# MaaniGhaffari/cvo-rgbd

Measured on AMD Instinct MI355X. Metric: frame-pair registrations/sec, higher is better.
Workload: dtype f32; 1 GPU; BASELINE configs[1] shape: 64 distinct synthetic 10000x10000 RGB-D cloud pairs (xyz + 5-dim colour) per align_many call, cvo align() to convergence, clouds resident in HBM; points_fixed=10000, points_moving=10000, mode=cvo, batch=64

## Files before the change

### cvo-rgbd_amd/csrc/cvo_capi.cpp

```cpp
#include "cvo_internal.h"

using namespace cvo_dev;
using namespace cvo_impl;

namespace cvo_impl {

int fail(cvo_hip_ctx *ctx, int code, const char *msg)
{
    if (ctx) ctx->err = msg;
    return code;
}

static std::atomic<bool> g_engine_debug{false};
bool engine_debug_on() { return g_engine_debug.load(std::memory_order_relaxed); }

namespace {
struct OptDef {
    const char *key;
    const char *env;
    int env_kind;
    double env_value;
};
const OptDef kOptions[] = {
    {"graph_capture", "CVO_HIP_GRAPH", 1, 1.0},           {"no_graph", "CVO_HIP_NO_GRAPH", 1, 1.0},
// ... 4 lines not shown
    {"async_builds", "CVO_HIP_NO_ASYNC", 1, 0.0},         {"list_pass_blocks", "CVO_HIP_PROC_BLOCKS", 2, 0.0},
    {"post_debug", "CVO_HIP_POST_DEBUG", 1, 1.0},         {"mailbox_timeout_s", "CVO_HIP_MAILBOX_TIMEOUT_S", 2, 0.0},
    {"candidate_records", "CVO_HIP_NO_CAND", 1, 0.0},     {"sync_upload", "CVO_HIP_SYNC_UPLOAD", 1, 1.0},
    {"engine_debug", "CVO_HIP_ENGINE_DEBUG", 1, 1.0},     {"one_launch_hand_over", "CVO_HIP_NO_CLOUD_ONE", 1, 0.0},
    {"small_calls_alone", "CVO_HIP_NO_ALONE", 1, 0.0},    {"fused_groups", "CVO_HIP_NO_FUSE", 1, 0.0},
    {"engines", "CVO_HIP_ENGINES_FORCE", 2, 0.0},         {"list_init", "CVO_HIP_LIST_INIT", 2, 0.0},
    {"kept_pack", "CVO_HIP_NO_PACK", 1, 0.0},             {"list_margin", "CVO_HIP_LIST_MARGIN", 2, 0.0},
    {"final_mirror", "CVO_HIP_NO_FINAL_MIRROR", 1, 0.0},  {"twist_on_shared_gpu", "CVO_HIP_TWIST_ON_SHARED_GPU", 1, 1.0},
    {"comm_debug", "CVO_HIP_COMM_DEBUG", 1, 1.0},         {"wait_policy", "CVO_HIP_WAIT_POLICY", 2, 0.0},
    {"acvo_runs", "CVO_HIP_NO_ACVO_RUN", 1, 0.0},         {"tail_alone", "CVO_HIP_TAIL_ALONE", 2, 0.0},         {"side_builds", "CVO_HIP_SIDE", 1, 1.0},
    {"run_build_at", "CVO_HIP_RUN_BUILD_AT", 2, 0.0},         {"alone_max", "CVO_HIP_ALONE_MAX", 2, 0.0},
    {"narrow_merge", "CVO_HIP_NARROW_MERGE", 1, 1.0},     {"narrow_blocks", "CVO_HIP_NARROW_BLOCKS", 2, 0.0},
    {"engine_crowd", "CVO_HIP_ENGINE_CROWD", 2, 0.0},     {"engine_merge_max", "CVO_HIP_ENGINE_MERGE_MAX", 2, 0.0},
    {"matches_combine", nullptr, 0, 0.0},                 {"scan_chunk", nullptr, 0, 0.0},
    {"record_narrow", "CVO_HIP_NO_RECORD_NARROW", 1, 0.0}, {"list_stale_max", "CVO_HIP_LIST_STALE_MAX", 2, 0.0},
};
void env_defaults(cvo_hip_ctx *ctx)
{
    for (const OptDef &d : kOptions) {
        if (!d.env) continue;
        const char *e = getenv(d.env);
        if (!e) continue;
        (void)apply_option(ctx, d.key, d.env_kind == 1 ? d.env_value : atof(e));
    }
}
}

int apply_option(cvo_hip_ctx *ctx, const char *key, double v)
{
    auto is = [&](const char *k) { return std::strcmp(key, k) == 0; };
// ... 23 lines not shown
    else if (is("post_debug")) o.post_debug = on;
    else if (is("mailbox_timeout_s")) { if (!(v > 0.0)) return CVO_HIP_ERR_INVALID; o.mailbox_timeout_s = v; }
    else if (is("candidate_records")) o.no_cand = !on;
    else if (is("sync_upload")) o.sync_upload = on;
    else if (is("engine_debug")) { o.engine_debug = on; if (on) g_engine_debug.store(true, std::memory_order_relaxed); }
    else if (is("one_launch_hand_over")) o.no_cloud_one = !on;
    else if (is("small_calls_alone")) o.no_alone = !on;
    else if (is("fused_groups")) o.no_fuse = !on;
    else if (is("engines")) { if (v < 0.0 || v > 8.0) return CVO_HIP_ERR_INVALID; o.engines_force = (int)v; }
    else if (is("list_init")) { if (v < 0.0) return CVO_HIP_ERR_INVALID; o.list_init = v; }
    else if (is("kept_pack")) o.no_pack = !on;
    else if (is("matches_combine")) o.matches_combine = on;
    else if (is("scan_chunk")) { if (v < 0.0 || v > (double)SCAN_CHUNK) return CVO_HIP_ERR_INVALID; o.scan_chunk = (int)v; }
    else if (is("list_margin")) { if (v > 4.0) return CVO_HIP_ERR_INVALID; o.list_margin = v < 0.0 ? -1.0f : (float)v; }
    else if (is("record_narrow")) o.record_narrow = on;
    else if (is("list_stale_max")) { if (!(v >= 1.0 && v <= 64.0)) return CVO_HIP_ERR_INVALID; o.list_stale_max = (float)v; }
    else if (is("final_mirror")) o.no_final_mirror = !on;
    else if (is("twist_on_shared_gpu")) o.twist_on_shared_gpu = on;
    else if (is("comm_debug")) o.comm_debug = on;
    else if (is("wait_policy")) { if (v < 0.0 || v > 2.0) return CVO_HIP_ERR_INVALID; o.wait_policy = (int)v; }
    else if (is("acvo_runs")) o.no_acvo_run = !on;
    else if (is("tail_alone")) { if (v < 0.0 || v > 32.0) return CVO_HIP_ERR_INVALID; o.tail_alone = (int)v; }
    else if (is("run_restart")) o.no_restart = !on;
    else if (is("side_builds")) o.no_side_builds = !on;
    else if (is("run_build_at")) { if (!(v > 0.0 && v <= 1.0)) return CVO_HIP_ERR_INVALID; o.run_build_at = (float)v; }
    else if (is("alone_max")) { if (v < 0.0 || v > 64.0) return CVO_HIP_ERR_INVALID; o.alone_max = (int)v; }
    else if (is("narrow_merge")) o.narrow_merge = on;
    else if (is("narrow_blocks")) { const int b = (int)v; if (b != 0 && b != 32 && b != 64) return CVO_HIP_ERR_INVALID; o.narrow_blocks = b; }
    else if (is("engine_crowd")) { if (v < 0.0) return CVO_HIP_ERR_INVALID; o.engine_crowd = (int)std::min(v, 1.0e6); }
    else if (is("engine_merge_max")) { if (v < 0.0 || v > 32.0) return CVO_HIP_ERR_INVALID; o.engine_merge_max = (int)v; }
// ... 725 lines not shown
    else if (is("engine_debug")) *value = o.engine_debug;
    else if (is("one_launch_hand_over")) *value = !o.no_cloud_one;
    else if (is("small_calls_alone")) *value = !o.no_alone;
    else if (is("fused_groups")) *value = !o.no_fuse;
    else if (is("engines")) *value = o.engines_force;
    else if (is("narrow_merge")) *value = o.narrow_merge;
    else if (is("narrow_blocks")) *value = o.narrow_blocks;
    else if (is("engine_crowd")) *value = o.engine_crowd;
    else if (is("engine_merge_max")) *value = o.engine_merge_max;
    else if (is("list_init")) *value = o.list_init;
    else if (is("kept_pack")) *value = !o.no_pack;
    else if (is("matches_combine")) *value = o.matches_combine;
    else if (is("scan_chunk")) *value = o.scan_chunk;
    else if (is("list_margin")) *value = o.list_margin;
    else if (is("record_narrow")) *value = o.record_narrow;
    else if (is("list_stale_max")) *value = o.list_stale_max;
    else if (is("final_mirror")) *value = !o.no_final_mirror;
    else if (is("twist_on_shared_gpu")) *value = o.twist_on_shared_gpu;
    else if (is("comm_debug")) *value = o.comm_debug;
    else if (is("wait_policy")) *value = o.wait_policy;
    else if (is("acvo_runs")) *value = !o.no_acvo_run;
    else if (is("tail_alone")) *value = o.tail_alone;
    else if (is("tail_handovers")) *value = (double)ctx->tail_handovers;
    else if (is("run_restart")) *value = !o.no_restart;
    else if (is("side_builds")) *value = !o.no_side_builds;
    else if (is("run_build_at")) *value = o.run_build_at;
    else if (is("side_builds_launched")) *value = (double)ctx->side_builds_launched;
    else if (is("alone_max")) *value = o.alone_max;
    else if (is("run_timeouts")) *value = (double)ctx->run_timeouts;
    else if (is("list_grows")) *value = (double)ctx->list_grows;
    else if (is("async_builds_named")) *value = (double)ctx->async_stats[0];
    else if (is("async_stalls")) *value = (double)ctx->async_stats[1];
    else if (is("run_aborts")) *value = (double)ctx->run_aborts;
    else if (is("engine_begins")) *value = (double)ctx->engine_begins;
    else if (is("engine_final_mirrored")) *value = (double)ctx->engine_final_mirrored;
    else if (is("engine_final_copied")) *value = (double)ctx->engine_final_copied;
    else if (is("no_run_backoff")) *value = ctx->no_run_backoff;
    else return CVO_HIP_ERR_INVALID;
    return CVO_HIP_OK;
}

long long cvo_hip_get_mirror_retries(void) { return mirror_retries().load(std::memory_order_relaxed); }

int cvo_hip_synchronize(cvo_hip_ctx *ctx)
{
// ... 9 lines not shown
```

### cvo-rgbd_amd/csrc/cvo_device.h

```cpp
#pragma once

#include <hip/hip_runtime.h>
#include <hip/hip_ext.h>
#include <stddef.h>
#include <stdint.h>

#include "cvo_hip.h"
#include "se3_math.hpp"

namespace cvo_dev {

constexpr int FEAT_STRIDE = 8;
constexpr int FEAT_INDEX_SLOT = 5;

constexpr int BLOCK = 256;
constexpr int TILES_PER_WAVE = 4;
constexpr int ROWS_PER_WAVE = 16 * TILES_PER_WAVE;
constexpr int ROWS_PER_TILE = 4 * ROWS_PER_WAVE;
constexpr float PAD_BIG = 1.0e30f;
constexpr int PROC_BLOCKS = 1024;
constexpr int PROC_WAVES = PROC_BLOCKS * 4;

constexpr int NSUB = 256;
constexpr int PROC_PARTS = PROC_BLOCKS / NSUB;
constexpr int TILE_STAGE = 128;
constexpr int DEAL_SHIFT = 2;
constexpr int PAIR_QUEUE = 128;
constexpr int SEG = 64;
constexpr int MAX_CSEG = 32;

typedef uint4 TileEntry;

enum ProcMode { PROC_FLOW = 0, PROC_STEP = 1, PROC_SELF = 2 };
enum ListId { LIST_XY = 0, LIST_XX = 1, LIST_YY = 2, LIST_KEPT = 3, LIST_XYB = 4, LIST_XXB = 5, LIST_YYB = 6,
              LIST_N = 7 };
CVO_HD int self_list_id(int l, int buf) { return buf ? LIST_XXB + l : LIST_XX + l; }

constexpr int NACC_FLOW = 9;
constexpr int NACC_STEP = 4;
constexpr int NACC_SELF = 2;
constexpr int NACC_MAX = 9;

constexpr int RED_FLOW = 0, RED_XX = 9, RED_YY = 11, RED_STEP = 13, RED_N = 17;

enum { RUNNING = 0, DONE_BREAK_A = 1, DONE_BREAK_B = 2, DONE_MAX_ITER = 3, NEED_BIGGER_LIST = 4,
       DONE_COMM_ERROR = 5,
// ... 64 lines not shown
    int32_t mode, max_iter;
    float ell_init, ell_min, ell_max_init;
    float sp, c_sp;
    float c, d, c_ell;
    float min_step, eps, eps_2;
    float log_sp_s2;
    float tau_c;
    float list_margin;
    int32_t async_xy;
    float build_at;
    int32_t async_self;
    float color_scale;
    float run_cand_cap;
    int32_t record_narrow;
    float list_stale_max;
    double s2_d, cs2_d, dl_step;
};

struct alignas(16) DevHead {
    float R[9], T[3];
    float ell, ell_max;
    float Rt[9], t[3];
    float used_Rt[9], used_t[3];
    KernConsts kc;
    float kc_ell, kc_pad_;
    float center[3];
    float xmax, y0max;
    float tauf[3];
    int32_t n_fixed;
    uint32_t pad0_;
    float list_r[3];
    int32_t list_ok[3];
    int32_t reuse[3];
    int32_t ck_nblk[3];
    float list_Rt[9], list_t[3];
    float rec_r;
    int32_t narrow;
    float rec_Rt[9], rec_t[3];
    int32_t list_stat[3];
    int32_t async_stat[2];
    int32_t rec_pad_;
    int32_t xy_active, xy_target, stall, xy_fresh;
    int32_t xy_ok[2];
    int32_t xy_ck[2];
    float xy_r[2];
    float tauf_build;
    float r_last;
    float xy_Rt[2][9], xy_t[2][3];
    int32_t sf_active[2], sf_target[2], sf_fresh[2];
    int32_t sf_ok[2][2];
    int32_t sf_ck[2][2];
    float sf_r[2][2];
    float sf_tauf_build[2];
    cvo_math::XiConsts xi;
    float omega[3], v[3];
    double dl;
// ... 216 lines not shown
}
CVO_HD float cull_slack(const float *t, const float cx, const float cy, const float cz, const float xmax, const float y0max)
{
    const float W = ((fabsf(cx) + fabsf(cy)) + fabsf(cz)) + (xmax + y0max);
    return (64.0f / 16777216.0f) * (3.0003f * W + ((fabsf(t[0]) + fabsf(t[1])) + fabsf(t[2])));
}

CVO_HD float reuse_slack(const float *t, const float *c, const float xmax, const float y0max, const float sides)
{
    const float W = ((fabsf(c[0]) + fabsf(c[1])) + fabsf(c[2])) + (xmax + y0max);
    const float S = 3.0003f * W + ((fabsf(t[0]) + fabsf(t[1])) + fabsf(t[2]));
    return 1.0e-4f * (1.0f + xmax + y0max) + sides * (22.0f / 16777216.0f) * S;
}

constexpr float LIST_LOOSE = 1.3f;
CVO_HD float pose_travel(const DevHead *s, const float *Rt0, const float *t0, const float ymax)
{
    float f2 = 0.0f, c2 = 0.0f;
    for (int r = 0; r < 3; ++r) {
        float dc = s->t[r] - t0[r];
        for (int q = 0; q < 3; ++q) {
            const float d = s->Rt[3 * r + q] - Rt0[3 * r + q];
            f2 += d * d;
            dc += d * s->center[q];
        }
        c2 += dc * dc;
    }
    return sqrtf(0.5f * f2) * 1.001f * ymax + sqrtf(c2);
}
CVO_HD void plan_lists(DevHead *s, DevHead *bulk, const bool store, const DevParams &p, const float r_now)
{
    const float ymax = s->y0max;
    const float slack_xx = reuse_slack(s->t, s->center, s->xmax, ymax, 0.0f), slack_xy = reuse_slack(s->t, s->center, s->xmax, ymax, 1.0f);
    const float wide_yy = slack_xy - slack_xx;
    const float margin = p.list_margin;
    const bool sync_xy = s->list_ok[LIST_XY] && !p.async_xy;
    const float travel = sync_xy ? pose_travel(s, s->list_Rt, s->list_t, ymax) : 0.0f;
#pragma unroll
    for (int l = 0; l < 3; ++l) {
        if (l == LIST_XY && p.async_xy) continue;
        if (l != LIST_XY && p.async_self) continue;
        if (l != LIST_XY && p.mode != CVO_HIP_MODE_ACVO) { s->reuse[l] = 1; continue; }
        const float slack = l == LIST_XX ? slack_xx : slack_xy;
        const float need = (r_now + (l == LIST_XY ? travel : 0.0f)) * 1.0001f + slack;
        const float lr = s->list_r[l];
        const float r0 = r_now * 1.0001f + slack;
        const float rb = r0 * (1.0f + margin);
        bool keep = margin > 0.0f && s->list_ok[l] && need <= lr;
        if (l == LIST_XY && p.record_narrow && keep && s->ck_nblk[LIST_XY] != 0) {
            const float tr = pose_travel(s, s->rec_Rt, s->rec_t, ymax);
            const float rr = s->rec_r;
            keep = (r_now + tr) * 1.0001f + slack <= rr && lr <= fmaxf(p.list_stale_max, LIST_LOOSE) * (1.0f + margin) * r0;
            s->narrow &= REC_BOUNDED;
            if (keep && !(rr <= LIST_LOOSE * (1.0f + margin) * r0)) {
                keep = (rb + tr) * 1.0001f + slack <= rr;
                if (keep) {
                    s->rec_r = rb * 1.000001f;
                    s->narrow = REC_NARROW | REC_BOUNDED;
                    s->list_stat[1] += 1;
                    if (store) {
                        for (int q = 0; q < 9; ++q) bulk->rec_Rt[q] = s->Rt[q];
                        for (int q = 0; q < 3; ++q) bulk->rec_t[q] = s->t[q];
                    }
                }
            }
        } else {
            keep = keep && lr <= LIST_LOOSE * (1.0f + margin) * r0;
// ... 447 lines not shown
    const float4 *pos_b;
    const float *feat_b;
    const float4 *seg_b;
    const float *tf;
    double *partials;
    double *out;
    KernConsts kc;
    int nseg_a, nseg_b;
    int nblk;
    int count;
};
void launch_pose_scan(const ScanArgs &a, int weight, hipStream_t s);

void launch_prepare(DevState *st, const DevParams &prm, hipStream_t s, uint32_t *build_masks = nullptr, const PrepareInit *init = nullptr);
void launch_prepare_many(const PrepareEntry *e, int n, hipStream_t s, uint32_t *build_masks);
void launch_filter(const FilterArgs &a, dim3 grid, hipStream_t s, hipEvent_t ev_start = nullptr,
                   hipEvent_t ev_stop = nullptr);
void launch_process(int mode, const ProcessArgs &a, hipStream_t s, hipEvent_t ev_start = nullptr,
                    hipEvent_t ev_stop = nullptr);
void launch_post_flow(const PostFlowArgs &a, hipStream_t s);
void launch_post_step(const PostStepArgs &a, hipStream_t s);
void launch_filter_group(const FilterArgs *a, int n, hipStream_t s);
void launch_process_group(int mode, const ProcessArgs *a, int n, hipStream_t s, hipEvent_t ev_start = nullptr,
                          hipEvent_t ev_stop = nullptr);
void launch_post_flow_group(const PostFlowArgs *a, int n, hipStream_t s);
void launch_post_step_group(const PostStepArgs *a, int n, hipStream_t s);
void launch_step_twist_group(const ProcessArgs *a, int n, hipStream_t s, hipEvent_t ev_start = nullptr,
                             hipEvent_t ev_stop = nullptr);
constexpr int STEP_TWIST_ROWS_DIV = 4;

// ... 21 lines not shown
```

### cvo-rgbd_amd/csrc/cvo_engine.cpp

```cpp
#include "cvo_internal.h"

using namespace cvo_dev;
using namespace cvo_impl;

namespace cvo_impl {

bool fusable(const cvo_hip_ctx *c) { return !c->profiling && !multi_rank(c) && !(c->prm.color_scale > 0.0f); }



struct EngineProfile {
    std::mutex mu;
    bool on = false;
    double flow_ms = 0.0, flow_slots = 0.0;
    long long flow_launches = 0;
    std::vector<float> dur_us, period_us;
    std::vector<int> slots;
};
EngineProfile *engine_profile()
{
    static EngineProfile *p = new EngineProfile;
    return p;
}

// ... 30 lines not shown
    struct Retire { hipEvent_t ev = nullptr; std::vector<AlignJob *> jobs; };
    std::vector<Retire> retiring;
    hipEvent_t ev[4] = {};
    std::vector<PrepareEntry> prep;
    long long launched = 0, checked = 0;
    int zdim = 0;
    bool crowded = true, use_graph = true, dirty = true, failed = false;
    int batch_len = kEngineBatch;
    bool narrow = false;
    bool narrow_merge = false;
    int narrow_blocks = 0;
    bool wind_down = false;
    std::vector<TLaunch> plan;
    struct FlowEv { hipEvent_t a, b; int live; };
    std::vector<FlowEv> flow_ev;
    long long n_batches[5] = {}, n_replans = 0, n_inserts = 0, n_sends = 0, n_prepares = 0, n_mirrored = 0, n_copied = 0;
    double t_replan = 0, t_insert = 0, t_launch = 0, t_finish = 0, t_wait = 0, t_collect = 0, t_idle_at = 0;
    static double now_ms() { return std::chrono::duration<double, std::milli>(std::chrono::steady_clock::now().time_since_epoch()).count(); }

    int create(int dev)
    {
        device = dev;
        if (hipSetDevice(dev) != hipSuccess) return -1;
        if (hipStreamCreateWithFlags(&s, hipStreamNonBlocking) != hipSuccess) return -1;
        if (tab.init(ENGINE_SLOTS, s) != 0) return -1;
        for (auto &e : ev)
            if (hipEventCreateWithFlags(&e, hipEventDisableTiming) != hipSuccess) return -1;
        return 0;
    }

    int live() const { int n = 0; for (AlignJob *j : member) n += j != nullptr; return n; }
// ... 88 lines not shown
            return CVO_HIP_OK;
        }
        member[z] = j;
        ops[z].clear();
        dirty = true;
        return CVO_HIP_OK;
    }

    int replan()
    {
        int n = 0;
        for (int z = 0; z < ENGINE_SLOTS; ++z) n += member[z] != nullptr;
        int zd = 1;
        while (zd < n) zd *= 2;
        if (n > 16 && n <= 24) zd = 24;
        for (int z = ENGINE_SLOTS - 1, hole = 0; z >= zd; --z) {
            if (!member[z]) continue;
            while (member[hole]) ++hole;
            member[hole] = member[z]; member[z] = nullptr;
            ops[hole].swap(ops[z]); ops[z].clear();
        }
        const bool regeom = zd != zdim;
        zdim = zd;
        const int nblk = (narrow && narrow_blocks > 0) ? std::min(narrow_blocks, nblk_for(zdim)) : nblk_for(zdim);
        int merge_max = 2;
        std::vector<const std::vector<RecOp> *> po;
        std::vector<Slot *> ps;
        for (int z = 0; z < ENGINE_SLOTS; ++z)
            if (member[z]) { merge_max = member[z]->ctx->opt.engine_merge_max; break; }
        for (int z = 0; z < ENGINE_SLOTS; ++z) {
// ... 239 lines not shown
                if (q + 1 < e->flow_ev.size() && hipEventElapsedTime(&gap, fe.a, e->flow_ev[q + 1].a) != hipSuccess) gap = 0.f;
                if (pr->dur_us.size() < (size_t)1 << 20) {
                    pr->dur_us.push_back(ms * 1e3f); pr->period_us.push_back(gap * 1e3f); pr->slots.push_back(fe.live);
                }
            }
        }
        for (auto &fe : e->flow_ev) {
            (void)hipEventDestroy(fe.a);
            (void)hipEventDestroy(fe.b);
        }
        e->flow_ev.clear();
    }
    std::lock_guard<std::mutex> lock(*engine_mutex());
    if (engine_debug_on())
        fprintf(stderr, "[cvo_hip] engine %p: batches at zdim 1/2/4/8/16: %lld %lld %lld %lld %lld, replans %lld, "
                "prepare launches %lld, final states mirrored %lld copied %lld, graph captures %lld hits %lld; host ms: insert %.2f replan %.2f launch %.2f collect %.2f finish %.2f wait %.2f\n",
                (void *)e, e->n_batches[0], e->n_batches[1], e->n_batches[2],
                e->n_batches[3], e->n_batches[4], e->n_replans, e->n_prepares, e->n_mirrored, e->n_copied, e->plans.captures, e->plans.hits,
                e->t_insert, e->t_replan, e->t_launch, e->t_collect, e->t_finish, e->t_wait);
    e->t_insert = e->t_replan = e->t_launch = e->t_collect = e->t_finish = e->t_wait = 0;
    for (long long &v : e->n_batches) v = 0;
    e->n_replans = e->n_prepares = e->n_mirrored = e->n_copied = 0;
    e->launched = e->checked = 0;
    e->in_use = false;
}


}

extern "C" {

int cvo_hip_align_many(cvo_hip_ctx **ctxs, cvo_hip_state **states, int *n_iters, int count)
{
    cvo_lock::Api api_guard;
    if (count < 0 || (count > 0 && (!ctxs || !states))) return CVO_HIP_ERR_INVALID;
    const bool dbg_many = engine_debug_on();
    const double t_many0 = Engine::now_ms();
// ... 224 lines not shown
```

### cvo-rgbd_amd/csrc/cvo_internal.h

```cpp
#pragma once
#include "cvo_hip.h"

#include <hip/hip_runtime.h>

#include <algorithm>
#include <atomic>
#include <chrono>
#include <cmath>
#include <cstddef>
#include <cstdint>
#include <cstdio>
#include <cstdlib>
#include <cstring>
#include <deque>
#include <memory>
#include <mutex>
#include <new>
#include <string>
#include <thread>
#include <vector>

#include "cvo_cloud.h"
#include "cvo_comm.h"
#include "cvo_device.h"
// ... 187 lines not shown
    bool no_side_builds = true;
    float run_build_at = 0.6f;
    bool no_restart = false;
    bool no_acvo_run = false;
    int tail_alone = 8;
    int alone_max = 0;
    int engines_force = 0;
    int narrow_blocks = 0;
    bool narrow_merge = false;
    int engine_crowd = 2;
    int engine_merge_max = 2;
    double list_init = 0.0;
    float list_margin = -1.0f;
    bool record_narrow = true;
    float list_stale_max = 3.0f;
    int run_cand = 0;
    double mailbox_timeout_s = 5.0;
    double run_timeout_ms = 0.0;
    int run_fault = 0;
    int wait_policy = 0;
};

struct cvo_hip_ctx {
    CtxOptions opt;
    int no_run_backoff = 0;
    long long side_builds_launched = 0;
    long long tail_handovers = 0;
    long long engine_begins = 0;
    long long engine_final_mirrored = 0;
    long long engine_final_copied = 0;
    long long run_aborts = 0;
    int list_stats[3] = {0, 0, 0};
    int async_stats[2] = {0, 0};
    long long list_grows = 0;
    long long run_timeouts = 0;
    int device = 0;
    hipStream_t stream = nullptr;
    bool own_stream = false;
    cvo_hip_params prm{};
    DevParams dprm{};
    Cloud fixed, moving;
    Cloud scratch_a, scratch_b;
    DevState *st = nullptr;
    DevHead *st2 = nullptr;
    bool head_mode = false;
    bool allow_head = true;
    DevState *st_host = nullptr;
// ... 125 lines not shown
inline bool runs_allowed(const cvo_hip_ctx *ctx) { return ctx->allow_run && ctx->no_run_backoff <= 0; }
const char *params_problem(const cvo_hip_params &p);
DevParams make_dev_params(const cvo_hip_params &p);
int cloud_ready(cvo_hip_ctx *ctx, Cloud &c);
int cloud_reserve(cvo_hip_ctx *ctx, Cloud &c, const float *xyz, const float *feat, int n, int layout);
int upload_cloud(cvo_hip_ctx *ctx, Cloud &c, const float *xyz, const float *feat, int n, int layout, bool on_device = false);
FilterPlan plan_filter(int nrows, int nb);
int ensure_buf(cvo_hip_ctx *ctx, DevBuf &b, size_t bytes);
int ensure_list(cvo_hip_ctx *ctx, int list, int nrows, int nb, double at_least);
void shard_ranges(const cvo_hip_ctx *ctx, int &rlo, int &rhi, int &slo, int &shi);
int fill_filter_geometry(cvo_hip_ctx *ctx, DevState *h);
int mailboxes_usable(cvo_hip_ctx *ctx);
bool host_reduce(const cvo_hip_ctx *ctx);
bool multi_rank(const cvo_hip_ctx *ctx);
DevParams loop_params(const cvo_hip_ctx *ctx);
hipStream_t loop_stream(const cvo_hip_ctx *ctx);
int enqueue_filter(cvo_hip_ctx *ctx, int list, const Cloud &ca, int row_lo, int row_hi, int tf_a, const Cloud &cb, int tf_b, int check_done);
int kept_format(const cvo_hip_ctx *ctx, unsigned *ebase);
KeptView kept_view(const cvo_hip_ctx *ctx);
int enqueue_process(cvo_hip_ctx *ctx, int mode, int list, DevBuf &part, const float4 *pos_a, const float *feat_a, int tf_a,
                    const float4 *pos_b, const float *feat_b, int tf_b, int first_counted, int check_done);
int drain_events(cvo_hip_ctx *ctx, int n_exec = -1, const DevState *fin = nullptr);
int reduce_over_ranks(cvo_hip_ctx *ctx, int off, int count);
int enqueue_flow(cvo_hip_ctx *ctx, bool tf_moving, int check_done, bool do_math, cvo_hip_trace *trace, int trace_cap);
int enqueue_step(cvo_hip_ctx *ctx, int check_done, bool do_math, cvo_hip_trace *trace, int trace_cap);
int check_overflow_and_grow(cvo_hip_ctx *ctx, bool *redo);
int prepare_buffers(cvo_hip_ctx *ctx);
int enqueue_iterations(cvo_hip_ctx *ctx, int count, int tag0, int trace_cap);
void drop_graphs(cvo_hip_ctx *ctx);
TLaunch mk_launch(int kernel, int q, unsigned gx, unsigned gz, unsigned smem = 0);
// ... 28 lines not shown
```

### cvo-rgbd_amd/csrc/cvo_job.cpp

```cpp
#include "cvo_internal.h"

using namespace cvo_dev;
using namespace cvo_impl;

namespace cvo_impl {

void decide_scheme(cvo_hip_ctx *ctx)
{
    const bool small_pair = (double)ctx->fixed.n * (double)ctx->moving.n <= 2.5e7;
    if (!ctx->proc_blocks_forced)
        ctx->proc_blocks = ctx->proc_blocks_default = small_pair ? PROC_BLOCKS / 2 : PROC_BLOCKS;
    ctx->use_async = ctx->allow_async && !ctx->crowded && !ctx->profiling && !multi_rank(ctx) &&
                     !(ctx->prm.color_scale > 0.0f) &&
                     (double)ctx->fixed.n * (double)ctx->moving.n <= 2.0e8;
    ctx->use_async_self = ctx->use_async && ctx->allow_async_self && ctx->lone &&
                          ctx->prm.mode == CVO_HIP_MODE_ACVO;
    const double npairs = (double)ctx->fixed.n * (double)ctx->moving.n;
    if (ctx->use_async_self && !ctx->proc_blocks_forced)
        ctx->proc_blocks = ctx->proc_blocks_default = npairs <= 6.0e7 ? PROC_BLOCKS / 8 : PROC_BLOCKS / 4;
    if (!ctx->proc_blocks_forced && !ctx->use_async_self && ctx->use_async && ctx->lone && ctx->allow_head &&
        ctx->prm.mode == CVO_HIP_MODE_CVO)
    {
        const bool runs = runs_allowed(ctx) && ctx->fixed.np <= 65536 && ctx->moving.np <= 65536;
        ctx->proc_blocks = ctx->proc_blocks_default =
// ... 177 lines not shown
    if (f.done == DONE_COMM_ERROR) {
        ctx->mail_broken = true;
        if (ctx->opt.comm_debug)
            fprintf(stderr, "[cvo_hip] rank %d of %d: exchange timed out at iteration k = %d (executed %d), mail_seq %llu, mail_snap %llu, slots %d, twist in launch %d\n",
                    ctx->mail_rank, ctx->mail_world, f.k, f.n_exec, (unsigned long long)f.mail_seq, (unsigned long long)f.mail_snap, f.n_slots,
                    (int)(ctx->plan.size() == 4));
        return fail(ctx, CVO_HIP_ERR_COMM, "mailbox all-reduce timed out: a peer rank never delivered its partial sums "
                                           "(the mailboxes must be created and connected again on every rank)");
    }
    if (f.done == DONE_RUN_TIMEOUT)
        return fail(ctx, CVO_HIP_ERR_RUN, "a resident run timed out and the registration could not be redone without runs");
    if (f.done == RUNNING || f.done == NEED_BIGGER_LIST)
        return fail(ctx, CVO_HIP_ERR_INVALID, "align loop ended without a verdict");
    const int executed = f.n_exec;
    for (int q = 0; q < 3; ++q) ctx->list_stats[q] = f.list_stat[q];
    for (int q = 0; q < 2; ++q) ctx->async_stats[q] = f.async_stat[q];
    if (j.trace_cap > 0 && executed > 0)
        HIP_TRY(ctx, hipMemcpy(j.trace, ctx->trace_dev,
                               (size_t)std::min(executed, j.trace_cap) * sizeof(cvo_hip_trace),
                               hipMemcpyDeviceToHost));
    if (executed > 0) cvo_math::tf_to_mat4(f.used_Rt, f.used_t, s->transform);
    std::memcpy(s->R, f.R, sizeof(s->R));
    std::memcpy(s->T, f.T, sizeof(s->T));
    s->ell = f.ell;
    s->ell_max = f.ell_max;
    s->iter = f.iter;
    std::memcpy(s->prev_transform, s->transform, sizeof(s->transform));
    cvo_math::mat4_mul(s->accum_transform, s->transform, s->accum_transform);
    float Rt[9], t[3];
    cvo_math::inverse_tf(s->R, s->T, Rt, t);
// ... 240 lines not shown
```

### cvo-rgbd_amd/csrc/cvo_kernels.hip

```cpp
#include <algorithm>
#include <atomic>
#include <cstdlib>

#include "cvo_device.h"
#include "cvo_pair.h"

namespace cvo_dev {

typedef float f32x4 __attribute__((ext_vector_type(4)));

__device__ __forceinline__ float mv_row(const float *m, float x, float y, float z)
{
    return (m[0] * x + m[1] * y) + m[2] * z;
}

constexpr int FILTER_KMAX = 64;
size_t filter_smem_bytes(int jt)
{
    return (size_t)jt * 16 + ROWS_PER_TILE * 16 + 4 * TILE_STAGE * sizeof(TileEntry) +
           FILTER_KMAX * 4 * 4;
}

__device__ __forceinline__ void flush_tiles(const TileEntry *stage, int n, int lane, unsigned rot, unsigned region,
                                            const FilterArgs &a, int list, TileEntry *tiles, const int par)
// ... 747 lines not shown
#else
        constexpr bool EPF = PIPE;
#endif
        TileEntry ahead = mine;
        for (unsigned eb = e0; eb < n; eb += 64u * stride) {
            if (eb != e0) mine = EPF ? ahead : tl[min(eb + (unsigned)lane * stride, a.subcap - 1)];
            if (EPF && eb + 64u * stride < n) ahead = tl[min(eb + (64u + (unsigned)lane) * stride, a.subcap - 1)];
            const unsigned left = (n - eb + stride - 1) / stride;
            const int cnt = (int)(left < 64u ? left : 64u);
            for (int k = 0; k < cnt; ++k) {
                const unsigned tx = (unsigned)__builtin_amdgcn_readlane((int)mine.x, k);
                const unsigned ty = (unsigned)__builtin_amdgcn_readlane((int)mine.y, k);
                const unsigned long long m =
                    (unsigned long long)(unsigned)__builtin_amdgcn_readlane((int)mine.z, k) |
                    ((unsigned long long)(unsigned)__builtin_amdgcn_readlane((int)mine.w, k) << 32);
                const unsigned r = ty >> 30, tcol = ty & 0x3fffffffu;
                if (__builtin_amdgcn_inverse_ballot_w64(m)) {
                    const unsigned below = __builtin_amdgcn_mbcnt_hi(
                        (unsigned)(m >> 32), __builtin_amdgcn_mbcnt_lo((unsigned)m, 0u));
                    pairq[qn + below] =
                        make_uint2(tx + (unsigned)(lane >> 4) * 4u + r, tcol + (unsigned)(lane & 15));
                }
                qn += __popcll(m);
                if (qn >= 64) {
                    qn -= 64;
                    run_batch(qn, 64);
                }
            }
        }
        sub += (unsigned)a.nblk; n = n_next; tl = tl_next; mine = mine_next;
        }
        if (qn > 0) run_batch(0, qn);
        if (MODE == PROC_FLOW && lane == 0) a.kept_cnt[wave] = nk;
        if (REC && lane == 0) hd.cand_cnt[wave] = co;
        if (lane == 0) acc[MODE == PROC_FLOW ? 8 : 1] = (double)nk;
        return true;
// ... 1165 lines not shown
    step_twist_body(a, head_mode ? (par ? st_a : st_b) : st_a, par, head_mode);
}

__global__ void __launch_bounds__(BLOCK) kt_post_flow(const Slot *__restrict__ tab, const int q)
{
    CVO_SLOT(tab);
    const PostFlowArgs a = CVO_ARG(PostFlowArgs, op[q].pf);
    post_flow_body(a);
}

__global__ void __launch_bounds__(BLOCK) kt_post_step(const Slot *__restrict__ tab, const int q)
{
    CVO_SLOT(tab);
    const PostStepArgs a = CVO_ARG(PostStepArgs, op[q].ps);
    post_step_body(a);
}

#define CVO_MERGED_KERNELS(SUFFIX, WAVES)                                                                  \
    __global__ void __launch_bounds__(BLOCK) __attribute__((amdgpu_waves_per_eu(WAVES, 8)))               \
    kt_flow_build##SUFFIX(const Slot *__restrict__ tab, const int q)                                       \
    {                                                                                                      \
        extern __shared__ __attribute__((aligned(16))) char smem[];                                        \
        CVO_SLOT(tab);                                                                                     \
        const int np = cs->op[q].np;                                                                       \
        if ((int)blockIdx.x < np) {                                                                        \
            const ProcessArgs &pa = CVO_ARG(ProcessArgs, op[q].p);                                         \
            process_body<PROC_FLOW, 0, false, false>(pa, blockIdx.x, smem, proc_head_global<PROC_FLOW>(pa, pa.st, 0)); \
            return;                                                                                        \
        }                                                                                                  \
        filter_body<false>(CVO_ARG(FilterArgs, op[q].f), blockIdx.x - (unsigned)np, (unsigned)cs->op[q].n0,       \
// ... 1410 lines not shown
```

### cvo-rgbd_amd/csrc/cvo_plan.cpp

```cpp
#include "cvo_internal.h"

using namespace cvo_dev;
using namespace cvo_impl;

namespace cvo_impl {

FilterPlan plan_filter(int nrows, int nb)
{
    FilterPlan p{};
    const int tiles = std::max(1, (nrows + ROWS_PER_TILE - 1) / ROWS_PER_TILE);
    const int want_blocks = 4096;
    const int chunks_want = std::max(1, (want_blocks + tiles / 2) / tiles);
    int jt = (nb + chunks_want - 1) / chunks_want;
    jt = std::max(jt, 64);
    jt = std::min(jt, 2048);
    jt = (jt + SEG - 1) & ~(SEG - 1);
    p.jt = jt;
    const int chunks = std::max(1, (nb + jt - 1) / jt);
    p.grid = dim3(chunks, tiles);
    return p;
}

int ensure_buf(cvo_hip_ctx *ctx, DevBuf &b, size_t bytes)
{
// ... 371 lines not shown
        } else if (ev.kind == LIST_XY) {
            ctx->prof.flow_ms += ms; ctx->prof.flow_launches++; ctx->prof.flow_pairs += ev.pairs;
        } else {
            ctx->prof.self_ms += ms; ctx->prof.self_launches++; ctx->prof.self_pairs += ev.pairs;
        }
        (void)hipEventDestroy(ev.a);
        (void)hipEventDestroy(ev.b);
    }
    ctx->events.clear();
    return CVO_HIP_OK;
}

bool host_reduce(const cvo_hip_ctx *ctx) { return !ctx->comm_table && (ctx->comm || ctx->user_allreduce); }
bool multi_rank(const cvo_hip_ctx *ctx) { return ctx->comm_table || ctx->comm || ctx->user_allreduce; }

DevParams loop_params(const cvo_hip_ctx *ctx)
{
    DevParams dp = ctx->dprm;
    dp.list_margin = ((double)ctx->fixed.n * (double)ctx->moving.n <= 2.0e8) ? 0.25f : 0.15f;
    if (ctx->prm.mode == CVO_HIP_MODE_ACVO && ctx->lone && ctx->use_async_self && runs_allowed(ctx) && !ctx->opt.no_acvo_run && ctx->allow_head &&
        (double)ctx->fixed.n * (double)ctx->moving.n <= 2.0e8)
        dp.list_margin = 0.5f;
    if (ctx->opt.list_margin >= 0.0f) dp.list_margin = ctx->opt.list_margin;
    dp.async_xy = ctx->use_async ? 1 : 0;
    dp.async_self = ctx->use_async_self ? 1 : 0;
    if (ctx->use_async && ctx->lone && ctx->allow_head && !multi_rank(ctx)) dp.build_at = 0.9f;
    if (ctx->use_async && ctx->lone && ctx->allow_head && runs_allowed(ctx) && !multi_rank(ctx) && ctx->prm.mode == CVO_HIP_MODE_CVO &&
        !(ctx->prm.color_scale > 0.0f) && !ctx->post_dbg && ctx->allow_merge && ctx->fixed.np <= 65536 && ctx->moving.np <= 65536 && !ctx->opt.no_cand)
        dp.run_cand_cap = (float)ctx->run_g_max * (float)(RUN_BLOCK * (RUN_R + RUN_L));
    dp.record_narrow = ctx->opt.record_narrow ? 1 : 0;
    dp.list_stale_max = ctx->opt.list_stale_max;
    return dp;
}

int reduce_over_ranks(cvo_hip_ctx *ctx, int off, int count)
{
    double *buf = reinterpret_cast<double *>(reinterpret_cast<char *>(ctx->st) +
                                             offsetof(DevState, red)) + off;
    if (ctx->comm_table) return CVO_HIP_OK;
    if (ctx->comm) {
        if (cvo_comm_allreduce(ctx->comm, buf, count, ctx->stream) != 0)
            return fail(ctx, CVO_HIP_ERR_COMM, cvo_comm_last_error(ctx->comm));
    } else if (ctx->user_allreduce) {
        if (ctx->user_allreduce(ctx->user_allreduce_arg, buf, count, (void *)ctx->stream) != 0)
            return fail(ctx, CVO_HIP_ERR_COMM, "user all-reduce failed");
    }
// ... 674 lines not shown
```

Baseline: 4384 registrations/s.

## Rebuild XY tile list from recorded candidates when engine batch width changes

When the batched engine changes its z-dimension, a new pair of kernels rebuilds each eligible slot's XY tile list directly from the recorded candidate pairs. It also adopts the record's radius and pose as the list's reference, so the next iteration avoids a full filter rebuild of the list. For engine slots it relaxes the list staleness bound, which keeps narrowed lists much longer. The cost is extra kernel launches at replan time, overflow handling that falls back to invalidating the list, and a risk of keeping over-wide lists that make the process kernel do more work.

Result: faster. 4436 registrations/s (median of 6 runs) (+1.2%).

```diff
diff --git a/cvo-rgbd_amd/csrc/cvo_capi.cpp b/cvo-rgbd_amd/csrc/cvo_capi.cpp
--- a/cvo-rgbd_amd/csrc/cvo_capi.cpp
+++ b/cvo-rgbd_amd/csrc/cvo_capi.cpp
@@ -42,6 +42,7 @@
     {"engine_crowd", "CVO_HIP_ENGINE_CROWD", 2, 0.0},     {"engine_merge_max", "CVO_HIP_ENGINE_MERGE_MAX", 2, 0.0},
     {"matches_combine", nullptr, 0, 0.0},                 {"scan_chunk", nullptr, 0, 0.0},
     {"record_narrow", "CVO_HIP_NO_RECORD_NARROW", 1, 0.0}, {"list_stale_max", "CVO_HIP_LIST_STALE_MAX", 2, 0.0},
+    {"tiles_from_record", "CVO_HIP_NO_TILES_FROM_RECORD", 1, 0.0}, {"tiles_from_record_cap", nullptr, 0, 0.0},
 };
 void env_defaults(cvo_hip_ctx *ctx)
 {
@@ -95,6 +96,8 @@
     else if (is("scan_chunk")) { if (v < 0.0 || v > (double)SCAN_CHUNK) return CVO_HIP_ERR_INVALID; o.scan_chunk = (int)v; }
     else if (is("list_margin")) { if (v > 4.0) return CVO_HIP_ERR_INVALID; o.list_margin = v < 0.0 ? -1.0f : (float)v; }
     else if (is("record_narrow")) o.record_narrow = on;
+    else if (is("tiles_from_record")) o.tiles_from_record = on;
+    else if (is("tiles_from_record_cap")) { if (v < 0.0 || v > 1.0e9) return CVO_HIP_ERR_INVALID; o.tiles_from_record_cap = (int)v; }
     else if (is("list_stale_max")) { if (!(v >= 1.0 && v <= 64.0)) return CVO_HIP_ERR_INVALID; o.list_stale_max = (float)v; }
     else if (is("final_mirror")) o.no_final_mirror = !on;
     else if (is("twist_on_shared_gpu")) o.twist_on_shared_gpu = on;
@@ -850,6 +853,8 @@
     else if (is("scan_chunk")) *value = o.scan_chunk;
     else if (is("list_margin")) *value = o.list_margin;
     else if (is("record_narrow")) *value = o.record_narrow;
+    else if (is("tiles_from_record")) *value = o.tiles_from_record;
+    else if (is("tiles_from_record_cap")) *value = o.tiles_from_record_cap;
     else if (is("list_stale_max")) *value = o.list_stale_max;
     else if (is("final_mirror")) *value = !o.no_final_mirror;
     else if (is("twist_on_shared_gpu")) *value = o.twist_on_shared_gpu;
@@ -865,6 +870,7 @@
     else if (is("alone_max")) *value = o.alone_max;
     else if (is("run_timeouts")) *value = (double)ctx->run_timeouts;
     else if (is("list_grows")) *value = (double)ctx->list_grows;
+    else if (is("tile_rebuilds")) *value = (double)ctx->tile_rebuilds;
     else if (is("async_builds_named")) *value = (double)ctx->async_stats[0];
     else if (is("async_stalls")) *value = (double)ctx->async_stats[1];
     else if (is("run_aborts")) *value = (double)ctx->run_aborts;
diff --git a/cvo-rgbd_amd/csrc/cvo_device.h b/cvo-rgbd_amd/csrc/cvo_device.h
--- a/cvo-rgbd_amd/csrc/cvo_device.h
+++ b/cvo-rgbd_amd/csrc/cvo_device.h
@@ -30,6 +30,17 @@
 constexpr int MAX_CSEG = 32;
 
 typedef uint4 TileEntry;
+CVO_HD void tile_pair(const unsigned x, const unsigned y, const unsigned bit, unsigned &i, unsigned &j)
+{
+    i = x + (bit >> 4) * 4u + (y >> 30);
+    j = (y & 0x3fffffffu) + (bit & 15u);
+}
+CVO_HD void tile_key(const unsigned i, const unsigned j, unsigned &x, unsigned &y, unsigned &bit)
+{
+    x = i & ~15u;
+    y = (j & ~15u) | ((i & 3u) << 30);
+    bit = (((i >> 2) & 3u) << 4) | (j & 15u);
+}
 
 enum ProcMode { PROC_FLOW = 0, PROC_STEP = 1, PROC_SELF = 2 };
 enum ListId { LIST_XY = 0, LIST_XX = 1, LIST_YY = 2, LIST_KEPT = 3, LIST_XYB = 4, LIST_XXB = 5, LIST_YYB = 6,
@@ -124,6 +135,7 @@
     float run_cand_cap;
     int32_t record_narrow;
     float list_stale_max;
+    float list_stale_engine;
     double s2_d, cs2_d, dl_step;
 };
 
@@ -149,7 +161,7 @@
     float rec_Rt[9], rec_t[3];
     int32_t list_stat[3];
     int32_t async_stat[2];
-    int32_t rec_pad_;
+    int32_t tile_rebuilds;
     int32_t xy_active, xy_target, stall, xy_fresh;
     int32_t xy_ok[2];
     int32_t xy_ck[2];
@@ -396,19 +408,28 @@
 }
 
 constexpr float LIST_LOOSE = 1.3f;
-CVO_HD float pose_travel(const DevHead *s, const float *Rt0, const float *t0, const float ymax)
+CVO_HD float pose_travel_between(const float *Rt1, const float *t1, const float *Rt0, const float *t0, const float *center, const float ymax)
 {
     float f2 = 0.0f, c2 = 0.0f;
     for (int r = 0; r < 3; ++r) {
-        float dc = s->t[r] - t0[r];
+        float dc = t1[r] - t0[r];
         for (int q = 0; q < 3; ++q) {
-            const float d = s->Rt[3 * r + q] - Rt0[3 * r + q];
+            const float d = Rt1[3 * r + q] - Rt0[3 * r + q];
             f2 += d * d;
-            dc += d * s->center[q];
+            dc += d * center[q];
         }
         c2 += dc * dc;
     }
     return sqrtf(0.5f * f2) * 1.001f * ymax + sqrtf(c2);
+}
+CVO_HD float pose_travel(const DevHead *s, const float *Rt0, const float *t0, const float ymax)
+{
+    return pose_travel_between(s->Rt, s->t, Rt0, t0, s->center, ymax);
+}
+CVO_HD bool record_covers_its_radius(const DevHead *s)
+{
+    const float tr = pose_travel_between(s->rec_Rt, s->rec_t, s->list_Rt, s->list_t, s->center, s->y0max);
+    return (s->rec_r + tr) * 1.0001f + reuse_slack(s->rec_t, s->center, s->xmax, s->y0max, 1.0f) <= s->list_r[LIST_XY];
 }
 CVO_HD void plan_lists(DevHead *s, DevHead *bulk, const bool store, const DevParams &p, const float r_now)
 {
@@ -432,7 +453,8 @@
         if (l == LIST_XY && p.record_narrow && keep && s->ck_nblk[LIST_XY] != 0) {
             const float tr = pose_travel(s, s->rec_Rt, s->rec_t, ymax);
             const float rr = s->rec_r;
-            keep = (r_now + tr) * 1.0001f + slack <= rr && lr <= fmaxf(p.list_stale_max, LIST_LOOSE) * (1.0f + margin) * r0;
+            const float stale = p.list_stale_engine > 0.0f ? p.list_stale_engine : p.list_stale_max;
+            keep = (r_now + tr) * 1.0001f + slack <= rr && lr <= fmaxf(stale, LIST_LOOSE) * (1.0f + margin) * r0;
             s->narrow &= REC_BOUNDED;
             if (keep && !(rr <= LIST_LOOSE * (1.0f + margin) * r0)) {
                 keep = (rb + tr) * 1.0001f + slack <= rr;
@@ -910,6 +932,7 @@
 
 void launch_prepare(DevState *st, const DevParams &prm, hipStream_t s, uint32_t *build_masks = nullptr, const PrepareInit *init = nullptr);
 void launch_prepare_many(const PrepareEntry *e, int n, hipStream_t s, uint32_t *build_masks);
+void launch_tiles_from_record(const Slot *tab, int q, unsigned gz, unsigned slot_mask, unsigned cap_limit, hipStream_t s);
 void launch_filter(const FilterArgs &a, dim3 grid, hipStream_t s, hipEvent_t ev_start = nullptr,
                    hipEvent_t ev_stop = nullptr);
 void launch_process(int mode, const ProcessArgs &a, hipStream_t s, hipEvent_t ev_start = nullptr,
diff --git a/cvo-rgbd_amd/csrc/cvo_engine.cpp b/cvo-rgbd_amd/csrc/cvo_engine.cpp
--- a/cvo-rgbd_amd/csrc/cvo_engine.cpp
+++ b/cvo-rgbd_amd/csrc/cvo_engine.cpp
@@ -68,7 +68,7 @@
     std::vector<TLaunch> plan;
     struct FlowEv { hipEvent_t a, b; int live; };
     std::vector<FlowEv> flow_ev;
-    long long n_batches[5] = {}, n_replans = 0, n_inserts = 0, n_sends = 0, n_prepares = 0, n_mirrored = 0, n_copied = 0;
+    long long n_batches[5] = {}, n_replans = 0, n_inserts = 0, n_sends = 0, n_prepares = 0, n_mirrored = 0, n_copied = 0, n_rebuilds = 0;
     double t_replan = 0, t_insert = 0, t_launch = 0, t_finish = 0, t_wait = 0, t_collect = 0, t_idle_at = 0;
     static double now_ms() { return std::chrono::duration<double, std::milli>(std::chrono::steady_clock::now().time_since_epoch()).count(); }
 
@@ -187,6 +187,22 @@
         int zd = 1;
         while (zd < n) zd *= 2;
         if (n > 16 && n <= 24) zd = 24;
+        if (zd != zdim && zdim > 0 && n > 0) {
+            unsigned mask = 0u, cap_limit = 0u;
+            for (int z = 0; z < std::min(zdim, (int)ENGINE_SLOTS); ++z)
+                if (member[z] && !ops[z].empty() && tiles_from_record_slot(member[z]->ctx)) {
+                    mask |= 1u << z;
+                    cap_limit = (unsigned)member[z]->ctx->opt.tiles_from_record_cap;
+                }
+            int q_flow = -1;
+            for (const TLaunch &l : plan)
+                if (l.kernel == TK_FLOW || l.kernel == TK_FLOW_D2) q_flow = l.q;
+            if (mask != 0u && q_flow >= 0) {
+                launch_tiles_from_record(tab.dev, q_flow, (unsigned)zdim, mask, cap_limit, s);
+                if (hipGetLastError() != hipSuccess) return CVO_HIP_ERR_HIP;
+                ++n_rebuilds;
+            }
+        }
         for (int z = ENGINE_SLOTS - 1, hole = 0; z >= zd; --z) {
             if (!member[z]) continue;
             while (member[hole]) ++hole;
@@ -456,13 +472,13 @@
     std::lock_guard<std::mutex> lock(*engine_mutex());
     if (engine_debug_on())
         fprintf(stderr, "[cvo_hip] engine %p: batches at zdim 1/2/4/8/16: %lld %lld %lld %lld %lld, replans %lld, "
-                "prepare launches %lld, final states mirrored %lld copied %lld, graph captures %lld hits %lld; host ms: insert %.2f replan %.2f launch %.2f collect %.2f finish %.2f wait %.2f\n",
+                "prepare launches %lld, tile-list rebuild launches %lld, final states mirrored %lld copied %lld, graph captures %lld hits %lld; host ms: insert %.2f replan %.2f launch %.2f collect %.2f finish %.2f wait %.2f\n",
                 (void *)e, e->n_batches[0], e->n_batches[1], e->n_batches[2],
-                e->n_batches[3], e->n_batches[4], e->n_replans, e->n_prepares, e->n_mirrored, e->n_copied, e->plans.captures, e->plans.hits,
+                e->n_batches[3], e->n_batches[4], e->n_replans, e->n_prepares, e->n_rebuilds, e->n_mirrored, e->n_copied, e->plans.captures, e->plans.hits,
                 e->t_insert, e->t_replan, e->t_launch, e->t_collect, e->t_finish, e->t_wait);
     e->t_insert = e->t_replan = e->t_launch = e->t_collect = e->t_finish = e->t_wait = 0;
     for (long long &v : e->n_batches) v = 0;
-    e->n_replans = e->n_prepares = e->n_mirrored = e->n_copied = 0;
+    e->n_replans = e->n_prepares = e->n_mirrored = e->n_copied = e->n_rebuilds = 0;
     e->launched = e->checked = 0;
     e->in_use = false;
 }
diff --git a/cvo-rgbd_amd/csrc/cvo_internal.h b/cvo-rgbd_amd/csrc/cvo_internal.h
--- a/cvo-rgbd_amd/csrc/cvo_internal.h
+++ b/cvo-rgbd_amd/csrc/cvo_internal.h
@@ -225,6 +225,8 @@
     float list_margin = -1.0f;
     bool record_narrow = true;
     float list_stale_max = 3.0f;
+    bool tiles_from_record = true;
+    int tiles_from_record_cap = 0;
     int run_cand = 0;
     double mailbox_timeout_s = 5.0;
     double run_timeout_ms = 0.0;
@@ -242,6 +244,7 @@
     long long engine_final_copied = 0;
     long long run_aborts = 0;
     int list_stats[3] = {0, 0, 0};
+    int tile_rebuilds = 0;
     int async_stats[2] = {0, 0};
     long long list_grows = 0;
     long long run_timeouts = 0;
@@ -397,6 +400,7 @@
 bool host_reduce(const cvo_hip_ctx *ctx);
 bool multi_rank(const cvo_hip_ctx *ctx);
 DevParams loop_params(const cvo_hip_ctx *ctx);
+bool tiles_from_record_slot(const cvo_hip_ctx *ctx);
 hipStream_t loop_stream(const cvo_hip_ctx *ctx);
 int enqueue_filter(cvo_hip_ctx *ctx, int list, const Cloud &ca, int row_lo, int row_hi, int tf_a, const Cloud &cb, int tf_b, int check_done);
 int kept_format(const cvo_hip_ctx *ctx, unsigned *ebase);
diff --git a/cvo-rgbd_amd/csrc/cvo_job.cpp b/cvo-rgbd_amd/csrc/cvo_job.cpp
--- a/cvo-rgbd_amd/csrc/cvo_job.cpp
+++ b/cvo-rgbd_amd/csrc/cvo_job.cpp
@@ -215,6 +215,7 @@
         return fail(ctx, CVO_HIP_ERR_INVALID, "align loop ended without a verdict");
     const int executed = f.n_exec;
     for (int q = 0; q < 3; ++q) ctx->list_stats[q] = f.list_stat[q];
+    ctx->tile_rebuilds = f.tile_rebuilds;
     for (int q = 0; q < 2; ++q) ctx->async_stats[q] = f.async_stat[q];
     if (j.trace_cap > 0 && executed > 0)
         HIP_TRY(ctx, hipMemcpy(j.trace, ctx->trace_dev,
diff --git a/cvo-rgbd_amd/csrc/cvo_kernels.hip b/cvo-rgbd_amd/csrc/cvo_kernels.hip
--- a/cvo-rgbd_amd/csrc/cvo_kernels.hip
+++ b/cvo-rgbd_amd/csrc/cvo_kernels.hip
@@ -785,12 +785,12 @@
                 const unsigned long long m =
                     (unsigned long long)(unsigned)__builtin_amdgcn_readlane((int)mine.z, k) |
                     ((unsigned long long)(unsigned)__builtin_amdgcn_readlane((int)mine.w, k) << 32);
-                const unsigned r = ty >> 30, tcol = ty & 0x3fffffffu;
                 if (__builtin_amdgcn_inverse_ballot_w64(m)) {
                     const unsigned below = __builtin_amdgcn_mbcnt_hi(
                         (unsigned)(m >> 32), __builtin_amdgcn_mbcnt_lo((unsigned)m, 0u));
-                    pairq[qn + below] =
-                        make_uint2(tx + (unsigned)(lane >> 4) * 4u + r, tcol + (unsigned)(lane & 15));
+                    unsigned pi, pj;
+                    tile_pair(tx, ty, (unsigned)lane, pi, pj);
+                    pairq[qn + below] = make_uint2(pi, pj);
                 }
                 qn += __popcll(m);
                 if (qn >= 64) {
@@ -1986,6 +1986,122 @@
     CVO_SLOT(tab);
     const PostStepArgs a = CVO_ARG(PostStepArgs, op[q].ps);
     post_step_body(a);
+}
+
+__device__ __forceinline__ bool tiles_from_record_wanted(const ProcessArgs &a, const DevState *st)
+{
+    if (!a.cand || !a.cand_cnt || a.async_xy || a.list != LIST_XY || a.kept_packed != 1 || a.weight != 0 || a.kept_wcap == 0u) return false;
+    if (st->done != RUNNING || !st->list_ok[LIST_XY]) return false;
+    const int ck = st->ck_nblk[LIST_XY];
+    if (ck == 0 || ck != a.nblk || ck < 64 || ck > PROC_BLOCKS || (ck & (ck - 1)) != 0) return false;
+    unsigned ovf = 0u;
+#pragma unroll
+    for (int l = 0; l < 8; ++l) ovf |= st->ovf[0][l];
+    if (ovf != 0u) return false;
+    return record_covers_its_radius(st);
+}
+
+__global__ void __launch_bounds__(BLOCK) kt_tiles_from_record(const Slot *__restrict__ tab, const int q, const unsigned slot_mask, const unsigned cap_limit)
+{
+    if (((slot_mask >> blockIdx.z) & 1u) == 0u) return;
+    CVO_SLOT(tab);
+    const ProcessArgs &a = CVO_ARG(ProcessArgs, op[q].p);
+    DevState *st = a.st;
+    if (!tiles_from_record_wanted(a, st)) return;
+    const int lane = threadIdx.x & 63;
+    const int wid = __builtin_amdgcn_readfirstlane((int)(threadIdx.x >> 6));
+    const unsigned d = blockIdx.x * 4u + (unsigned)wid;
+    if (d >= (unsigned)NSUB) return;
+    const unsigned nblk = (unsigned)a.nblk, wcap = a.kept_wcap, subcap = min(a.subcap, cap_limit);
+    const unsigned nsrc = nblk / (NSUB / 4);
+    TileEntry *out_tl = const_cast<TileEntry *>(a.tiles) + (size_t)d * subcap;
+    unsigned out = 0;
+    unsigned cx = 0u, cy = 0u;
+    unsigned long long cm = 0ull;
+    for (unsigned k = 0; k < nsrc; ++k) {
+        const unsigned slice = nblk >= (unsigned)NSUB ? (d + (unsigned)NSUB * (k >> 2)) * 4u + (k & 3u)
+                                                      : (d % nblk) * 4u + d / nblk + ((unsigned)NSUB / nblk) * k;
+        unsigned n = a.cand_cnt[slice];
+        if (n > wcap) n = wcap;
+        const uint2 *src = a.cand + (size_t)slice * wcap;
+        for (unsigned b0 = 0; b0 < n; b0 += 64u) {
+            const bool live = b0 + (unsigned)lane < n;
+            const unsigned last = min(n - b0, 64u) - 1u;
+            unsigned x = 0xffffffffu - (unsigned)lane, y = 0u, bit = 0u;
+            if (live) {
+                const uint2 e = src[b0 + (unsigned)lane];
+                tile_key(e.x & 0xffffu, e.x >> 16, x, y, bit);
+            }
+            unsigned long long m = live ? 1ull << bit : 0ull;
+            const unsigned x_dn = (unsigned)__shfl_up((int)x, 1, 64), y_dn = (unsigned)__shfl_up((int)y, 1, 64);
+            const unsigned x_up = (unsigned)__shfl_down((int)x, 1, 64), y_up = (unsigned)__shfl_down((int)y, 1, 64);
+            int head = (lane == 0 || x_dn != x || y_dn != y) ? 1 : 0;
+            const bool tail = lane == 63 || x_up != x || y_up != y;
+            const unsigned long long heads = __ballot(head != 0);
+            const bool first_run = (heads & ((2ull << lane) - 1ull)) == 1ull;
+#pragma unroll
+            for (int s = 1; s < 64; s <<= 1) {
+                const unsigned lo = (unsigned)__shfl_up((int)(unsigned)m, s, 64), hi = (unsigned)__shfl_up((int)(unsigned)(m >> 32), s, 64);
+                const int head_o = __shfl_up(head, s, 64);
+                if (lane >= s) {
+                    if (!head) m |= ((unsigned long long)hi << 32) | lo;
+                    head |= head_o;
+                }
+            }
+            const unsigned x0 = (unsigned)__builtin_amdgcn_readfirstlane((int)x), y0 = (unsigned)__builtin_amdgcn_readfirstlane((int)y);
+            const bool joins = cm != 0ull && x0 == cx && y0 == cy;
+            if (joins && first_run) m |= cm;
+            if (cm != 0ull && !joins) {
+                if (lane == 0 && out < subcap) out_tl[out] = make_uint4(cx, cy, (unsigned)cm, (unsigned)(cm >> 32));
+                out += 1u;
+            }
+            const bool emit = live && tail && (unsigned)lane < last;
+            const unsigned long long em = __ballot(emit);
+            if (emit) {
+                const unsigned pos = out + __builtin_amdgcn_mbcnt_hi((unsigned)(em >> 32), __builtin_amdgcn_mbcnt_lo((unsigned)em, 0u));
+                if (pos < subcap) out_tl[pos] = make_uint4(x, y, (unsigned)m, (unsigned)(m >> 32));
+            }
+            out += (unsigned)__popcll(em);
+            cx = (unsigned)__builtin_amdgcn_readlane((int)x, (int)last);
+            cy = (unsigned)__builtin_amdgcn_readlane((int)y, (int)last);
+            cm = (unsigned long long)(unsigned)__builtin_amdgcn_readlane((int)(unsigned)m, (int)last) |
+                 ((unsigned long long)(unsigned)__builtin_amdgcn_readlane((int)(unsigned)(m >> 32), (int)last) << 32);
+        }
+    }
+    if (cm != 0ull) {
+        if (lane == 0 && out < subcap) out_tl[out] = make_uint4(cx, cy, (unsigned)cm, (unsigned)(cm >> 32));
+        out += 1u;
+    }
+    if (lane == 0) st->sub[LIST_XY][d] = out;
+}
+
+__global__ void __launch_bounds__(BLOCK) kt_tiles_from_record_head(const Slot *__restrict__ tab, const int q, const unsigned slot_mask, const unsigned cap_limit)
+{
+    if (((slot_mask >> blockIdx.z) & 1u) == 0u) return;
+    CVO_SLOT(tab);
+    const ProcessArgs &a = CVO_ARG(ProcessArgs, op[q].p);
+    DevState *st = a.st;
+    if (!tiles_from_record_wanted(a, st)) return;
+    static_assert(BLOCK == NSUB, "a thread per sub-list");
+    const int over = __syncthreads_or(st->sub[LIST_XY][threadIdx.x] > min(a.subcap, cap_limit) ? 1 : 0);
+    if (threadIdx.x != 0) return;
+    if (over) {
+        st->list_ok[LIST_XY] = 0;
+        st->ck_nblk[LIST_XY] = 0;
+        st->ovf[0][LIST_XY] = 1u;
+        return;
+    }
+    st->list_r[LIST_XY] = st->rec_r;
+    for (int k = 0; k < 9; ++k) st->list_Rt[k] = st->rec_Rt[k];
+    for (int k = 0; k < 3; ++k) st->list_t[k] = st->rec_t[k];
+    st->tile_rebuilds += 1;
+}
+
+void launch_tiles_from_record(const Slot *tab, int q, unsigned gz, unsigned slot_mask, unsigned cap_limit, hipStream_t s)
+{
+    if (cap_limit == 0u) cap_limit = 0xffffffffu;
+    hipLaunchKernelGGL(kt_tiles_from_record, dim3(NSUB / 4, 1, gz), dim3(BLOCK), 0, s, tab, q, slot_mask, cap_limit);
+    hipLaunchKernelGGL(kt_tiles_from_record_head, dim3(1, 1, gz), dim3(BLOCK), 0, s, tab, q, slot_mask, cap_limit);
 }
 
 #define CVO_MERGED_KERNELS(SUFFIX, WAVES)                                                                  \
diff --git a/cvo-rgbd_amd/csrc/cvo_plan.cpp b/cvo-rgbd_amd/csrc/cvo_plan.cpp
--- a/cvo-rgbd_amd/csrc/cvo_plan.cpp
+++ b/cvo-rgbd_amd/csrc/cvo_plan.cpp
@@ -409,6 +409,12 @@
 bool host_reduce(const cvo_hip_ctx *ctx) { return !ctx->comm_table && (ctx->comm || ctx->user_allreduce); }
 bool multi_rank(const cvo_hip_ctx *ctx) { return ctx->comm_table || ctx->comm || ctx->user_allreduce; }
 
+bool tiles_from_record_slot(const cvo_hip_ctx *ctx)
+{
+    return ctx->opt.tiles_from_record && ctx->opt.record_narrow && !ctx->lone && !ctx->use_async && !multi_rank(ctx) && !ctx->opt.no_cand &&
+           !(ctx->prm.color_scale > 0.0f) && ctx->fixed.np <= 65536 && ctx->moving.np <= 65536;
+}
+
 DevParams loop_params(const cvo_hip_ctx *ctx)
 {
     DevParams dp = ctx->dprm;
@@ -425,6 +431,7 @@
         dp.run_cand_cap = (float)ctx->run_g_max * (float)(RUN_BLOCK * (RUN_R + RUN_L));
     dp.record_narrow = ctx->opt.record_narrow ? 1 : 0;
     dp.list_stale_max = ctx->opt.list_stale_max;
+    dp.list_stale_engine = tiles_from_record_slot(ctx) ? 1.0e6f : 0.0f;
     return dp;
 }
 
```
